# vita-epfl/CrowdNav

Measured on NVIDIA H100. Metric: env-steps/sec at 5 humans × batched envs; 500-case success/collision parity, higher is better.
Workload: dtype f64 state + f32 ORCA solver

## Files before the change

crowdnav_b200/csrc/orca_spec.cuh:

```cuda
#pragma once
#include "orca_device.cuh"

namespace orca {

template <int M> struct RegLines { V2 p[M], d[M]; };

template <int M>
ORCA_HD __forceinline__ int neighbour_order(const float (&dsq)[M], const bool (&inr)[M], const int (&id)[M], int (&src)[M])
{
    static_assert(M <= 10, "3 bits per position in a 32-bit word");
    int rank[M];
    #pragma unroll
    for (int c = 0; c < M; ++c) rank[c] = 0;
    #pragma unroll
    for (int c = 1; c < M; ++c) {
        #pragma unroll
        for (int cc = 0; cc < c; ++cc) {
            const bool le = dsq[cc] <= dsq[c];
            rank[c] += (inr[cc] && le) ? 1 : 0;
            rank[cc] += (inr[c] && !le) ? 1 : 0;
        }
    }
    int nl = 0; unsigned packed = 0u;
    #pragma unroll
    for (int c = 0; c < M; ++c) if (inr[c]) { packed |= (unsigned)id[c] << (3 * rank[c]); ++nl; }
    #pragma unroll
    for (int kk = 0; kk < M; ++kk) src[kk] = (int)((packed >> (3 * kk)) & 7u);
    return nl;
}

ORCA_HD __forceinline__ void make_line_sel(V2 p, V2 v, float r, V2 po, V2 vo, float ro, float inv_th, float inv_dt,
                                              V2 &point, V2 &dir)
{
    const V2 rel_pos = po - p;
    const V2 rel_vel = v - vo;
    const float dist_sq = abssq(rel_pos);
    const float comb_r = r + ro;
    const float comb_r_sq = sqr(comb_r);
    V2 u;
    if (dist_sq > comb_r_sq) {
        const V2 w = rel_vel - inv_th * rel_pos;
        const float w_len_sq = abssq(w);
        const float dot1 = dot(w, rel_pos);
        const float w_len = sqrtf(w_len_sq);
        const V2 unit_w = vdiv(w, w_len);
        const V2 dir_c = mk(unit_w.y, -unit_w.x);
        const V2 u_c = (comb_r * inv_th - w_len) * unit_w;
        const float leg = sqrtf(dist_sq - comb_r_sq);
        const bool left = det(rel_pos, w) > 0.0f;
        const V2 num_l = mk(rel_pos.x * leg - rel_pos.y * comb_r, rel_pos.x * comb_r + rel_pos.y * leg);
        const V2 num_r = mk(rel_pos.x * leg + rel_pos.y * comb_r, -rel_pos.x * comb_r + rel_pos.y * leg);
        const V2 q = vdiv(left ? num_l : num_r, dist_sq);
        const V2 dir_l = left ? q : -q;
        const float dot2 = dot(rel_vel, dir_l);
        const V2 u_l = dot2 * dir_l - rel_vel;
        const bool cutoff = dot1 < 0.0f && sqr(dot1) > comb_r_sq * w_len_sq;
        dir = cutoff ? dir_c : dir_l;
        u = cutoff ? u_c : u_l;
    } else {
        const V2 w = rel_vel - inv_dt * rel_pos;
        const float w_len = sqrtf(abssq(w));
        const V2 unit_w = vdiv(w, w_len);
        dir = mk(unit_w.y, -unit_w.x);
        u = (comb_r * inv_dt - w_len) * unit_w;
    }
    point = v + 0.5f * u;
}

template <int M, int CNT>
ORCA_HD __forceinline__ void lp1_all(const RegLines<M> &R, const bool (&valid)[M], float radius, V2 opt, bool dir_opt,
                                        V2 (&cand)[M], bool (&feas)[M])
{
    #pragma unroll
    for (int i = 0; i < CNT; ++i) {
        const V2 lp = R.p[i], ld = R.d[i];
        const float dp = dot(lp, ld);
        const float disc = sqr(dp) + sqr(radius) - abssq(lp);
        const float sq = sqrtf(disc);
        float t_left = -dp - sq, t_right = -dp + sq;
        bool bad = disc < 0.0f;
        #pragma unroll
        for (int j = 0; j < i; ++j) {
            const float den = det(ld, R.d[j]);
            const float num = det(R.d[j], lp - R.p[j]);
            const bool use = valid[j];
            const bool par = fabsf(den) <= kEps;
            const bool live_pair = use && !par;
            const float t = (live_pair ? num : 1.0f) / (live_pair ? den : 1.0f);
            bad = bad || (use && par && num < 0.0f);
            const bool right = use && !par && den >= 0.0f, leftb = use && !par && den < 0.0f;
            t_right = (right && t < t_right) ? t : t_right;
            t_left = (leftb && t_left < t) ? t : t_left;
        }
        feas[i] = !bad && !(t_left > t_right);
        if (dir_opt) {
            cand[i] = (dot(opt, ld) > 0.0f) ? (lp + t_right * ld) : (lp + t_left * ld);
        } else {
            const float t = dot(ld, opt - lp);
            const float tc = (t < t_left) ? t_left : ((t > t_right) ? t_right : t);
            cand[i] = lp + tc * ld;
        }
    }
}

template <int M, int CNT>
ORCA_HD __forceinline__ int lp2_scan(const RegLines<M> &R, const bool (&valid)[M], int count, const V2 (&cand)[M], const bool (&feas)[M],
                                        V2 init, V2 &result)
{
    result = init;
    int fail = count;
    #pragma unroll
    for (int i = 0; i < CNT; ++i) {
        const bool viol = (i < count) && (fail == count) && valid[i] && det(R.d[i], R.p[i] - result) > 0.0f;
        if (viol) { if (!feas[i]) fail = i; else result = cand[i]; }
    }
    return fail;
}

ORCA_HD __forceinline__ V2 lp2_init(V2 opt, float radius)
{
    if (abssq(opt) > sqr(radius)) { const V2 nv = normalize(opt); return mk(nv.x * radius, nv.y * radius); }
    return opt;
}

ORCA_HD __forceinline__ float int_bits(int i) { float f; __builtin_memcpy(&f, &i, sizeof f); return f; }
ORCA_HD __forceinline__ int bits_int(float f) { int i; __builtin_memcpy(&i, &f, sizeof i); return i; }

template <int M>
struct Lp3Queue {
    static constexpr int kLines = M, kRows = 4 * M + 3;
    float *base;
    int stride;
    ORCA_HD __forceinline__ Lines lines(int col) const { return { base + col, stride }; }
    ORCA_HD __forceinline__ int n(int col) const { return bits_int(base[(4 * M + 0) * stride + col]); }
    ORCA_HD __forceinline__ int fail(int col) const { return bits_int(base[(4 * M + 1) * stride + col]); }
    ORCA_HD __forceinline__ float radius(int col) const { return base[(4 * M + 2) * stride + col]; }
    ORCA_HD __forceinline__ void put(int col, const RegLines<M> &R, int nl, int fail, float radius) const
    {
        #pragma unroll
        for (int kk = 0; kk < M; ++kk) lines(col).set(kk, R.p[kk], R.d[kk]);
        base[(4 * M + 0) * stride + col] = int_bits(nl); base[(4 * M + 1) * stride + col] = int_bits(fail);
        base[(4 * M + 2) * stride + col] = radius;
    }
};

#define ORCA_LP3_SUBPROBLEM_LANE(Q, COL, I, P, R2, RS, C) do {                                                         \
        const orca::Lines lq_ = (Q).lines(COL);                                                                          \
        const int qn_ = (Q).n(COL);                                                                                      \
        bool ok_ = false; orca::V2 r_ = orca::mk(0.f, 0.f);                                                             \
        if ((Q).kLines > 1 && (I) < qn_) ok_ = orca::lp3_subproblem(lq_, (I), (Q).radius(COL), (P), r_);                \
        (R2)[C] = r_.x; (R2)[(RS) + (C)] = r_.y; (R2)[2 * (RS) + (C)] = ok_ ? 1.0f : 0.0f;                             \
    } while (0)
#define ORCA_LP3_SCAN_LANE(Q, COL, RES, R2, RS, C) do {                                                                \
        const int qn_ = (Q).n(COL), qf_ = (Q).fail(COL);                                                                 \
        const float qr_ = (Q).radius(COL);                                                                               \
        orca::lp3_outer_scan((Q).lines(COL), qn_, qf_, qr_, (RES), [&](int ii_, orca::V2 &r_) {                         \
            const int src_ = (C) + (ii_ - 1);                                                                            \
            r_ = orca::mk((R2)[src_], (R2)[(RS) + src_]);                                                                \
            return (R2)[2 * (RS) + src_] != 0.0f;                                                                        \
        });                                                                                                              \
    } while (0)

template <int M>
ORCA_HD __forceinline__ void insert_sorted(float dd, int j, float (&td)[M], int (&tj)[M])
{
    #pragma unroll
    for (int kk = M - 1; kk >= 0; --kk) {
        const int km = kk > 0 ? kk - 1 : 0;
        const bool lt = dd < td[kk];
        const bool ltp = (kk > 0) && (dd < td[km]);
        td[kk] = ltp ? td[km] : (lt ? dd : td[kk]);
        tj[kk] = ltp ? tj[km] : (lt ? j : tj[kk]);
    }
}

}
```

crowdnav_b200/csrc/step_multi.cuh:

```cuda
#pragma once
#include "step_flat.cuh"
#include "rotate.cuh"

namespace cs {

#ifndef CS_MULTI_WARPS
#define CS_MULTI_WARPS 30
#endif

#define CS_PHASES 8
#ifdef CS_PHASE_PROBE
static __device__ unsigned long long g_phase[2][CS_PHASES + 1];
#define CS_PROBE_INIT unsigned ph_acc[CS_PHASES] = {}; long long ph_t = clock64();
#define CS_PROBE(i) do { const long long t_ = clock64(); ph_acc[i] += (unsigned)(t_ - ph_t); ph_t = t_; } while (0)
#define CS_PROBE_FLUSH(robot, steps) do { if ((threadIdx.x & 31) == 0) {                                                    \
        for (int i_ = 0; i_ < CS_PHASES; ++i_) atomicAdd(&g_phase[(robot) ? 1 : 0][i_], (unsigned long long)ph_acc[i_]);    \
        atomicAdd(&g_phase[(robot) ? 1 : 0][CS_PHASES], (unsigned long long)(steps)); } } while (0)
#else
#define CS_PROBE_INIT
#define CS_PROBE(i) do { } while (0)
#define CS_PROBE_FLUSH(robot, steps) do { } while (0)
#endif

template <int N, int M, bool ROBOT>
__device__ __forceinline__ orca::V2 multi_solve(const KParams &k, const float4 *s_view, const float *s_rview, int ebase, int a,
                                                bool solves, double2 pos, double2 goal, double v_pref, orca::V2 p, orca::V2 v,
                                                float r, const float *s_rl, orca::RegLines<N> &Rq, int &nl_out, int &fail_out,
                                                float &max_speed_out)
{
    using namespace orca;
    const V2 pref = pref_velocity(pos, goal);
    const float max_speed = (float)v_pref;

    float dsq[M]; bool inr[M]; int jj[M], src[M];
    #pragma unroll
    for (int c = 0; c < M; ++c) {
        const int j = ROBOT ? c : ((c < N - 1) ? ((c < a) ? c : c + 1) : N);
        jj[c] = j;
        const float4 q = s_view[ebase + j];
        dsq[c] = abssq(p - mk(q.x, q.y));
        inr[c] = solves && (k.max_neighbors > 0) && dsq[c] < sqr(k.neighbor_dist);
    }
    int nl = neighbour_order<M>(dsq, inr, jj, src);
    nl = nl < k.max_neighbors ? nl : k.max_neighbors;

    constexpr int T = 32 * (N + 1);
    if (ROBOT) asm volatile("barrier.sync 1, %0;" :: "r"(T) : "memory");
    RegLines<M> R; bool valid[M];
    #pragma unroll
    for (int kk = 0; kk < M; ++kk) {
        valid[kk] = kk < nl;
        R.p[kk] = mk(0.f, 0.f); R.d[kk] = mk(0.f, 0.f);
        if (valid[kk]) {
            if (ROBOT) {
                const int c = (ebase / (N + 1)) * N + src[kk];
                R.p[kk] = mk(s_rl[0 * T + c], s_rl[1 * T + c]); R.d[kk] = mk(s_rl[2 * T + c], s_rl[3 * T + c]);
            } else {
                const int sl = ebase + src[kk];
                const float4 q = s_view[sl];
                make_line_sel(p, v, r, mk(q.x, q.y), mk(q.z, q.w), s_rview[sl], k.inv_time_horizon, k.inv_time_step, R.p[kk], R.d[kk]);
            }
        }
    }

    V2 cand[M]; bool feas[M];
    lp1_all<M, M>(R, valid, max_speed, pref, false, cand, feas);
    V2 nv = mk(0.f, 0.f);
    fail_out = lp2_scan<M, M>(R, valid, nl, cand, feas, lp2_init(pref, max_speed), nv);
    #pragma unroll
    for (int kk = 0; kk < N; ++kk) { Rq.p[kk] = (kk < M) ? R.p[kk] : mk(0.f, 0.f); Rq.d[kk] = (kk < M) ? R.d[kk] : mk(0.f, 0.f); }
    nl_out = nl; max_speed_out = max_speed;
    return nv;
}

template <int E>
__device__ __forceinline__ float *rec_vpref_smem()
{
    __shared__ float s_vp[E];
    return s_vp;
}

template <int E>
__device__ __forceinline__ float *rec_theta_smem()
{
    __shared__ float s_th[E];
    return s_th;
}

template <bool ROT = false>
__device__ __forceinline__ void rec_row(const crowdsim_record &rec, int B, int N, int s, int e, int a, double2 hp, double2 hv,
                                        double hr, double2 rp, double2 rv, double2 rg, double rr, float rvp, float rth = 0.f)
{
    float c, sn, rot, dg, rvx, rvy;
    rotate_self((float)rp.x, (float)rp.y, (float)rv.x, (float)rv.y, (float)rg.x, (float)rg.y, c, sn, rot, dg, rvx, rvy);
    float row[13];
    rotate_row(row, (float)rp.x, (float)rp.y, (float)rr, rvp, ROT ? (rth - rot) : 0.f, dg, rvx, rvy, c, sn, (float)hp.x,
               (float)hp.y, (float)hv.x, (float)hv.y, (float)hr);
    float *o = rec.rows + (((size_t)s * B + e) * N + a) * 13;
    #pragma unroll
    for (int i = 0; i < 13; ++i) o[i] = row[i];
}

__device__ __forceinline__ void rec_map_state(const crowdsim_record_maps &m, int B, int N, int s, int e, int a, double2 hp, double2 hv)
{
    const size_t i = ((size_t)s * B + e) * N + a;
    st2(m.h_pos, i, hp); st2(m.h_vel, i, hv);
}

template <int N, bool VIS, bool REC, bool ROT = false, bool ARR = false, bool MET = false>
__global__ void __launch_bounds__(32 * (N + 1), CS_MULTI_WARPS / (N + 1))
step_multi_kernel(const __grid_constant__ StepArgs A)
{
    static_assert(REC || !ROT, "unicycle rows are a recording variant");
    static_assert(!(REC && ARR), "arrivals are stamped by the rollout kernels only");
    static_assert(!(REC && MET), "metrics are measured by the rollout kernels only");
    static_assert(N >= 2 && N <= 5, "small crowds with at least two humans (N = 1 runs n single-step launches)");
    using namespace orca;
    CS_RES_BEGIN
    constexpr int E = 32, L = N + 1, T = 32 * L;
    constexpr int MH = VIS ? N : N - 1;
    constexpr int SUB = N - 1;
    constexpr int IPW = 32 / SUB;
    constexpr int QC = IPW * L;
    constexpr int QF = Lp3Queue<N>::kRows + 1;
    constexpr int PV = (4 * SUB > 10) ? 4 * SUB : 10;
    __shared__ float s_q[QF][QC];
    __shared__ __align__(16) float s_pv[PV][T];
    __shared__ __align__(16) float s_r2[3][T];
    __shared__ double2 s_pos[T], s_vel[T];
    __shared__ double2 s_goal[T];
    __shared__ double s_rad[T];
    __shared__ float2 s_nv[T];
    __shared__ RobotRec s_rr[E];
    __shared__ uint8_t s_pre[E];
    __shared__ int s_qcount;
    constexpr unsigned PRE_TIMEOUT = 1, PRE_GOAL = 2, PRE_READY = 4, PRE_WANT = 8;
    float4 *const s_view = reinterpret_cast<float4 *>(&s_pv[0][0]);
    float *const s_radh = s_pv[4], *const s_radr = s_pv[5];
    const Lp3Queue<N> Q = { &s_q[0][0], QC };

    const KParams &k = A.k;
    const int tid = threadIdx.x;
    const bool is_robot = tid >= 32 * N;
    const int le = is_robot ? tid - 32 * N : tid / N;
    const int a = is_robot ? N : tid - le * N;
    const int slot_me = le * L + a;
    const int e = blockIdx.x * E + le;
    const bool env_ok = e < A.B;
    const size_t hi = (size_t)e * N + a;
    if (tid == 0) s_qcount = 0;

    double2 pos = make_double2(0, 0), vel = pos, goal = make_double2(3, 4), attr = make_double2(0.3, 1.0);
    uint8_t act_flag = 1;
    if (env_ok) {
        if (A.st.active) act_flag = A.st.active[e];
        if (!is_robot) {
            pos = ld2(A.st.h_pos, hi); vel = ld2(A.st.h_vel, hi); goal = ld2(A.st.h_goal, hi); attr = ld2(A.st.h_attr, hi);
        } else {
            pos = ld2(A.st.r_pos, e); vel = ld2(A.st.r_vel, e); goal = ld2(A.st.r_goal, e); attr = ld2(A.st.r_attr, e);
            RobotRec r0 = {}; r0.ep_c = -1;
            r0.gtime = A.st.g_time[e];
            if (A.has_ep) { r0.ep_t = A.ep.ep_steps[e]; r0.ep_ret = A.ep.ep_return[e]; r0.ep_tc = A.ep.ep_too_close[e]; r0.ep_mds = A.ep.ep_min_dist_sum[e]; r0.ep_c = A.ep.ep_case[e]; }
            if (A.has_ar) r0.want = A.ar.want[e];
            s_rr[le] = r0;
            if constexpr (ROT) rec_theta_smem<E>()[le] = (float)A.st.r_theta[e];
            if constexpr (MET) met_acc_smem<E>()[le] = met_load(A.met, e);
        }
    }
    if constexpr (MET) { if (is_robot) met_hh_smem<E>()[le] = 0; }
    s_goal[tid] = goal;
    RobotRec &rr = s_rr[le];
    bool arrived = false;
    if constexpr (ARR) { if (env_ok && !is_robot) arrived = A.arr.h_arrival[hi] != 0.0; }

    bool dirty_kin = false, dirty_scene = false;
    bool release = false;
    const double dt = k.time_step;
    CS_PROBE_INIT

    #pragma unroll 1
    for (int s = 0; ; ++s) {
    const bool live = env_ok && (act_flag != 0);
    const float fpx = (float)pos.x, fpy = (float)pos.y, fvx = (float)vel.x, fvy = (float)vel.y;
    const float frh = orca_radius(attr.x, k.human_safety_space);
    const float frr = orca_radius(attr.x, k.robot_safety_space);
    s_view[slot_me] = make_float4(fpx, fpy, fvx, fvy); s_radh[slot_me] = frh; s_radr[slot_me] = frr;
    s_pos[tid] = pos; s_vel[tid] = vel; s_rad[tid] = attr.x;
    if constexpr (REC) { if (is_robot) rec_vpref_smem<E>()[le] = (float)attr.y; }
    const bool work = live || (is_robot && env_ok && A.has_ar && rr.want != 0);
    const int go = __syncthreads_or(s < A.n_steps && work);
    if (release) { st_release_u8(A.ar.n_state + e, CROWDSIM_SLOT_EMPTY); release = false; }
    if (!go) {
        if constexpr (REC) { if (is_robot && env_ok) for (int s2 = s; s2 < A.n_steps; ++s2) A.rec.code[(size_t)s2 * A.B + e] = CROWDSIM_REC_NONE; }
        CS_PROBE_FLUSH(is_robot, s);
        break;
    }
    CS_PROBE(0);
    if constexpr (REC) {
        if (!is_robot && live) {
            const int rt = 32 * N + le;
            if constexpr (ROT)
                rec_row<true>(A.rec, A.B, N, s, e, a, pos, vel, attr.x, s_pos[rt], s_vel[rt], s_goal[rt], s_rad[rt],
                              rec_vpref_smem<E>()[le], rec_theta_smem<E>()[le]);
            else
                rec_row(A.rec, A.B, N, s, e, a, pos, vel, attr.x, s_pos[rt], s_vel[rt], s_goal[rt], s_rad[rt], rec_vpref_smem<E>()[le]);
            if (A.recm.h_pos) rec_map_state(A.recm, A.B, N, s, e, a, pos, vel);
        }
    }

    const V2 p = mk(fpx, fpy), v = mk(fvx, fvy);
    if (!is_robot) {
        const int rs = le * L + N;
        const float4 q = s_view[rs];
        V2 lp, ld;
        make_line_sel(mk(q.x, q.y), mk(q.z, q.w), s_radr[rs], p, v, frr, k.inv_time_horizon, k.inv_time_step, lp, ld);
        s_pv[6][tid] = lp.x; s_pv[7][tid] = lp.y; s_pv[8][tid] = ld.x; s_pv[9][tid] = ld.y;
        asm volatile("barrier.arrive 1, %0;" :: "r"(T) : "memory");
    }
    RegLines<N> R; int nl, fail; float max_speed;
    V2 nv = is_robot ? multi_solve<N, N, true>(k, s_view, s_radr, le * L, N, live, pos, s_goal[tid], attr.y, p, v, frr, s_pv[6], R, nl, fail, max_speed)
                     : multi_solve<N, MH, false>(k, s_view, s_radh, le * L, a, live, pos, s_goal[tid], attr.y, p, v, frh, s_pv[6], R, nl, fail, max_speed);

    const bool pending = live && fail < nl;
    int slot = pending ? atomicAdd(&s_qcount, 1) : -1;
    if (slot >= QC) {
        float lq[4 * N], lp[4 * SUB];
        #pragma unroll
        for (int kk = 0; kk < N; ++kk) { lq[4 * kk + 0] = R.p[kk].x; lq[4 * kk + 1] = R.p[kk].y; lq[4 * kk + 2] = R.d[kk].x; lq[4 * kk + 3] = R.d[kk].y; }
        const Lines Lq = { lq, 1 }, Pq = { lp, 1 };
        lp3(Lq, nl, fail, max_speed, Pq, nv);
        slot = -1;
    } else if (slot >= 0) {
        Q.put(slot, R, nl, fail, max_speed); s_q[QF - 1][slot] = __int_as_float(tid);
    }
    s_nv[tid] = make_float2(nv.x, nv.y);
    uint8_t sst = CROWDSIM_SLOT_EMPTY;
    double disc = 0.0;
    if (is_robot && env_ok) {
        if (A.has_ar) sst = ld_relaxed_u8(A.ar.n_state + e);
        if (A.has_ep && live) { const int t = rr.ep_t; disc = (t < A.ep.discount_len) ? A.ep.discount[t] : 0.0; }
    }
    CS_PROBE(1);
    const int cnt = __syncthreads_count(slot >= 0);
    CS_PROBE(2);
    if (cnt > 0) {
        if (tid == 0) s_qcount = 0;
        const int lane = tid & 31, item = (tid >> 5) * IPW + lane / SUB, i = lane % SUB + 1;
        const bool mine = lane < IPW * SUB && item < cnt;
        if (mine) { const Lines Pq = { &s_pv[0][tid], T }; ORCA_LP3_SUBPROBLEM_LANE(Q, item, i, Pq, &s_r2[0][0], T, tid); }
        __syncwarp();
        if (mine && i == 1) {
            const int owner = __float_as_int(s_q[QF - 1][item]);
            const float2 r0 = s_nv[owner];
            V2 res = mk(r0.x, r0.y);
            ORCA_LP3_SCAN_LANE(Q, item, res, &s_r2[0][0], T, tid);
            s_nv[owner] = make_float2(res.x, res.y);
        }
        __syncthreads();
        if (slot >= 0) { const float2 q = s_nv[tid]; nv = mk(q.x, q.y); }
    }
    pos = s_pos[tid]; vel = s_vel[tid];
    CS_PROBE(3);

    double *const s_cl = reinterpret_cast<double *>(&s_r2[0][0]);
    bool timeout = false, reaching_goal = false;
    int arr_c = -1;
    if (!is_robot) {
        if (live) {
            const int rt = 32 * N + le;
            const float2 rv = s_nv[rt];
            s_cl[tid] = swept_clearance(pos, vel, s_pos[rt], make_double2((double)rv.x, (double)rv.y), attr.x, s_rad[rt], dt);
            if constexpr (MET) {
                int c = 0;
                #pragma unroll
                for (int j = 1; j < N; ++j) if (j > a) c += hh_overlap(pos, attr.x, s_pos[le * N + j], s_rad[le * N + j]) ? 1 : 0;
                if (c) atomicAdd(&met_hh_smem<E>()[le], c);
            }
            const double hx = (double)nv.x, hy = (double)nv.y;
            pos = make_double2(pos.x + hx * dt, pos.y + hy * dt); vel = make_double2(hx, hy);
            dirty_kin = true;
            if constexpr (ARR) {
                arr_c = rr.ep_c;
                const double2 g = s_goal[tid];
                if (!arrived && norm2(pos.x - g.x, pos.y - g.y) < attr.x) { A.arr.h_arrival[hi] = rr.gtime + dt; arrived = true; }
            }
        }
    } else if (env_ok) {
        if (live) {
            const double npx = pos.x + (double)nv.x * dt, npy = pos.y + (double)nv.y * dt;
            const double2 goal = s_goal[tid];
            reaching_goal = norm2(npx - goal.x, npy - goal.y) < attr.x;
            timeout = rr.gtime >= k.time_limit - 1;
        }
        s_pre[le] = (uint8_t)((timeout ? PRE_TIMEOUT : 0u) | (reaching_goal ? PRE_GOAL : 0u) |
                              (sst == CROWDSIM_SLOT_READY ? PRE_READY : 0u) | (rr.want != 0 ? PRE_WANT : 0u));
    }
    CS_PROBE(4);
    __syncthreads();
    CS_PROBE(5);
    if (!is_robot) {
        if (env_ok) {
            const unsigned pf = s_pre[le];
            bool done = false;
            if (live) {
                bool collision = false;
                #pragma unroll
                for (int i = 0; i < N; ++i) collision |= s_cl[le * N + i] < 0;
                done = (pf & PRE_TIMEOUT) || collision || (pf & PRE_GOAL);
                if (done && A.has_ep && A.st.active && !A.has_ar) act_flag = 0;
                if constexpr (ARR) {
                    if (done && arr_c >= 0) arr_snap_human(A, arr_c, N, a, pos, vel, s_goal[tid], attr, arrived ? A.arr.h_arrival[hi] : 0.0);
                }
            }
            if (A.has_ar && ((live && done) || (!live && (pf & PRE_WANT)))) {
                act_flag = (pf & PRE_READY) ? 1 : 0;
                if (act_flag) {
                    (void)ld_acquire_u8(A.ar.n_state + e);
                    pos = ld2_cg(A.ar.n_h_pos, hi); vel = make_double2(0, 0); s_goal[tid] = ld2_cg(A.ar.n_h_goal, hi); attr = ld2_cg(A.ar.n_h_attr, hi);
                    dirty_kin = true; dirty_scene = true;
                    if constexpr (ARR) { A.arr.h_arrival[hi] = 0.0; arrived = false; }
                }
            }
        }
        CS_PROBE(6);
    } else {
        if (env_ok) {
            bool done = false;
            if (live) {
                const double ax = (double)nv.x, ay = (double)nv.y;
                double dmin = __longlong_as_double(0x7ff0000000000000LL); bool collision = false;
                #pragma unroll
                for (int i = 0; i < N; ++i) {
                    const double ci = s_cl[le * N + i];
                    if (!collision) { if (ci < 0) collision = true; else if (ci < dmin) dmin = ci; }
                }
                const double npx = pos.x + ax * dt, npy = pos.y + ay * dt;
                if constexpr (MET) {
                    int &hh = met_hh_smem<E>()[le];
                    met_add(met_acc_smem<E>()[le], pos, make_double2(npx, npy), dmin, hh);
                    hh = 0;
                }
                const double gtime = rr.gtime;
                const int t_rec = rr.ep_t;
                double reward;
                const int info = reward_ladder(timeout, collision, reaching_goal, dmin, k, dt, reward);
                done = ends_episode(info);
                pos = make_double2(npx, npy); vel = make_double2(ax, ay);
                const double ntime = gtime + dt;
                rr.gtime = ntime;
                rr.o_act = vel; rr.o_reward = reward; rr.o_dmin = dmin; rr.o_done = done ? 1 : 0; rr.o_info = info; rr.any_live = 1;
                dirty_kin = true;
                if (A.has_ep) {
                    const crowdsim_episodes &ep = A.ep;
                    int ep_t = rr.ep_t, ep_tc = rr.ep_tc; double ep_ret = rr.ep_ret, ep_mds = rr.ep_mds;
                    ep_ret = ep_ret + disc * reward; ep_t += 1;
                    if (info == CROWDSIM_INFO_DANGER) { ep_tc += 1; ep_mds += dmin; }
                    rr.ep_t = ep_t; rr.ep_tc = ep_tc; rr.ep_ret = ep_ret; rr.ep_mds = ep_mds;
                    rr.dirty_ep = 1;
                    if (done) {
                        const int ep_c = rr.ep_c;
                        if (ep_c >= 0) {
                            ep.res_info[ep_c] = (uint8_t)info; ep.res_steps[ep_c] = ep_t;
                            ep.res_time[ep_c] = (info == CROWDSIM_INFO_TIMEOUT) ? k.time_limit : ntime;
                            ep.res_return[ep_c] = ep_ret; ep.res_too_close[ep_c] = ep_tc; ep.res_min_dist_sum[ep_c] = ep_mds;
                            if (ep.res_final_rpos) st2(ep.res_final_rpos, ep_c, pos);
                            if constexpr (ARR) { if (A.arr.snap_r_vel) st2(A.arr.snap_r_vel, ep_c, vel); }
                            if constexpr (MET) met_result(A.met, ep_c, met_acc_smem<E>()[le]);
                        }
                        if (A.st.active && !A.has_ar) { A.st.active[e] = 0; act_flag = 0; }
                    }
                }
                if constexpr (REC) {
                    const size_t ri = (size_t)s * A.B + e;
                    A.rec.reward[ri] = reward; A.rec.t[ri] = t_rec;
                    A.rec.code[ri] = !done ? CROWDSIM_REC_LIVE : (info == CROWDSIM_INFO_TIMEOUT) ? CROWDSIM_REC_DROPPED : CROWDSIM_REC_STORED;
                }
            } else if constexpr (REC) {
                A.rec.code[(size_t)s * A.B + e] = CROWDSIM_REC_NONE;
            }
            if (A.has_ar) {
                const bool finished = live && done, parked = !live && rr.want != 0;
                if (finished || parked) {
                    if (sst == CROWDSIM_SLOT_READY) {
                        (void)ld_acquire_u8(A.ar.n_state + e);
                        pos = make_double2(0.0, -A.ar.circle_radius); s_goal[tid] = make_double2(0.0, A.ar.circle_radius);
                        vel = make_double2(0, 0); attr = make_double2(A.ar.robot_radius, A.ar.robot_v_pref);
                        rr.gtime = 0.0;
                        if (A.st.r_theta) A.st.r_theta[e] = CS_PI / 2;
                        if constexpr (ROT) rec_theta_smem<E>()[le] = (float)A.st.r_theta[e];
                        if (A.has_ep) { rr.ep_t = 0; rr.ep_ret = 0.0; rr.ep_tc = 0; rr.ep_mds = 0.0; rr.ep_c = __ldcg(A.ar.n_case + e); rr.dirty_ep = 1; rr.new_case = 1; }
                        if constexpr (MET) met_acc_smem<E>()[le] = met_fresh();
                        act_flag = 1; A.st.active[e] = 1; rr.want = 0; A.ar.want[e] = 0;
                        dirty_kin = true; dirty_scene = true; release = true;
                    } else {
                        act_flag = 0; A.st.active[e] = 0;
                        const uint8_t want = (sst == CROWDSIM_SLOT_EXHAUSTED) ? 0 : 1;
                        rr.want = want; A.ar.want[e] = want;
                    }
                }
            }
        }
        CS_PROBE(6);
    }
    }

    if (env_ok) {
        if (!is_robot) {
            if (dirty_kin) {
                st2(A.st.h_pos, hi, pos); st2(A.st.h_vel, hi, vel);
                if (A.io.obs32) reinterpret_cast<float4 *>(A.io.obs32)[hi] = make_float4((float)pos.x, (float)pos.y, (float)vel.x, (float)vel.y);
            }
            if (dirty_scene) { st2(A.st.h_goal, hi, s_goal[tid]); st2(A.st.h_attr, hi, attr); }
        } else {
            if (dirty_kin) { st2(A.st.r_pos, e, pos); st2(A.st.r_vel, e, vel); A.st.g_time[e] = rr.gtime; }
            if (dirty_scene) { st2(A.st.r_goal, e, s_goal[tid]); st2(A.st.r_attr, e, attr); }
            if (rr.any_live) {
                if (A.io.action_out) st2(A.io.action_out, e, rr.o_act);
                A.io.reward[e] = rr.o_reward; A.io.dmin[e] = rr.o_dmin; A.io.done[e] = rr.o_done; A.io.info[e] = (uint8_t)rr.o_info;
            }
            if (A.has_ep && rr.dirty_ep) {
                A.ep.ep_steps[e] = rr.ep_t; A.ep.ep_return[e] = rr.ep_ret; A.ep.ep_too_close[e] = rr.ep_tc; A.ep.ep_min_dist_sum[e] = rr.ep_mds;
                if (rr.new_case) A.ep.ep_case[e] = rr.ep_c;
                if constexpr (MET) met_store(A.met, e, met_acc_smem<E>()[le]);
            }
        }
    }
    CS_RES_END(CS_RES_STEP);
}

}
```

Baseline: 1.338 billion.

## Share symmetric pairwise ORCA core terms between human pairs via shared-memory table

Splits ORCA line construction into a symmetric pair core (overlap/cutoff decision, leg length and reciprocal, with flags packed into sign bits) and a per-agent finish. Each human pair's core is now computed once and written to a shared-memory table for both agents, so the sqrt and divide are not repeated per direction. Human neighbour lines are then built from the table. This adds a named barrier across the human threads, extra shared-memory traffic and a dependence on the core being exactly symmetric. It also aliases s_r2 and the table into the s_pv shared-memory allocation to save space.

```diff
diff --git a/crowdnav_b200/csrc/orca_spec.cuh b/crowdnav_b200/csrc/orca_spec.cuh
--- a/crowdnav_b200/csrc/orca_spec.cuh
+++ b/crowdnav_b200/csrc/orca_spec.cuh
@@ -67,6 +67,58 @@
     point = v + 0.5f * u;
 }
 
+ORCA_HD __forceinline__ float int_bits(int i) { float f; __builtin_memcpy(&f, &i, sizeof f); return f; }
+ORCA_HD __forceinline__ int bits_int(float f) { int i; __builtin_memcpy(&i, &f, sizeof i); return i; }
+
+ORCA_HD __forceinline__ V2 pair_core(V2 p, V2 v, float r, V2 po, V2 vo, float ro, float inv_th, float inv_dt)
+{
+    const V2 rel_pos = po - p;
+    const V2 rel_vel = v - vo;
+    const float dist_sq = abssq(rel_pos);
+    const float comb_r = r + ro;
+    const float comb_r_sq = sqr(comb_r);
+    const bool overlap = !(dist_sq > comb_r_sq);
+    const V2 w = rel_vel - (overlap ? inv_dt : inv_th) * rel_pos;
+    const float w_len_sq = abssq(w);
+    const float dot1 = dot(w, rel_pos);
+    const bool circle = overlap || (dot1 < 0.0f && sqr(dot1) > comb_r_sq * w_len_sq);
+    const bool left = det(rel_pos, w) > 0.0f;
+    const float len = sqrtf(circle ? w_len_sq : dist_sq - comb_r_sq);
+    const float inv = 1.0f / (circle ? len : dist_sq);
+    return mk(circle ? -len : len, (circle ? overlap : left) ? -inv : inv);
+}
+
+ORCA_HD __forceinline__ void line_from_core(V2 c, V2 p, V2 v, float r, V2 po, V2 vo, float ro, float inv_th, float inv_dt,
+                                            V2 &point, V2 &dir)
+{
+    const bool circle = bits_int(c.x) < 0, flag = bits_int(c.y) < 0;
+    const float len = fabsf(c.x), inv = fabsf(c.y);
+    const V2 rel_pos = po - p;
+    const V2 rel_vel = v - vo;
+    const float comb_r = r + ro;
+    const float k = (circle && flag) ? inv_dt : inv_th;
+    const V2 w = rel_vel - k * rel_pos;
+    const V2 unit_w = mk(w.x * inv, w.y * inv);
+    const V2 dir_c = mk(unit_w.y, -unit_w.x);
+    const V2 u_c = (comb_r * k - len) * unit_w;
+    const V2 num_l = mk(rel_pos.x * len - rel_pos.y * comb_r, rel_pos.x * comb_r + rel_pos.y * len);
+    const V2 num_r = mk(rel_pos.x * len + rel_pos.y * comb_r, -rel_pos.x * comb_r + rel_pos.y * len);
+    const V2 n = flag ? num_l : num_r;
+    const V2 q = mk(n.x * inv, n.y * inv);
+    const V2 dir_l = flag ? q : -q;
+    const float dot2 = dot(rel_vel, dir_l);
+    const V2 u_l = dot2 * dir_l - rel_vel;
+    dir = circle ? dir_c : dir_l;
+    const V2 u = circle ? u_c : u_l;
+    point = v + 0.5f * u;
+}
+
+ORCA_HD __forceinline__ void make_line_core(V2 p, V2 v, float r, V2 po, V2 vo, float ro, float inv_th, float inv_dt,
+                                            V2 &point, V2 &dir)
+{
+    line_from_core(pair_core(p, v, r, po, vo, ro, inv_th, inv_dt), p, v, r, po, vo, ro, inv_th, inv_dt, point, dir);
+}
+
 template <int M, int CNT>
 ORCA_HD __forceinline__ void lp1_all(const RegLines<M> &R, const bool (&valid)[M], float radius, V2 opt, bool dir_opt,
                                         V2 (&cand)[M], bool (&feas)[M])
@@ -123,9 +175,6 @@
     return opt;
 }
 
-ORCA_HD __forceinline__ float int_bits(int i) { float f; __builtin_memcpy(&f, &i, sizeof f); return f; }
-ORCA_HD __forceinline__ int bits_int(float f) { int i; __builtin_memcpy(&i, &f, sizeof i); return i; }
-
 template <int M>
 struct Lp3Queue {
     static constexpr int kLines = M, kRows = 4 * M + 3;
diff --git a/crowdnav_b200/csrc/step_multi.cuh b/crowdnav_b200/csrc/step_multi.cuh
--- a/crowdnav_b200/csrc/step_multi.cuh
+++ b/crowdnav_b200/csrc/step_multi.cuh
@@ -22,11 +22,18 @@
 #define CS_PROBE_FLUSH(robot, steps) do { } while (0)
 #endif
 
+template <int S>
+__device__ __forceinline__ float2 *pair_table_smem()
+{
+    __shared__ float2 s_pt[S];
+    return s_pt;
+}
+
 template <int N, int M, bool ROBOT>
 __device__ __forceinline__ orca::V2 multi_solve(const KParams &k, const float4 *s_view, const float *s_rview, int ebase, int a,
                                                 bool solves, double2 pos, double2 goal, double v_pref, orca::V2 p, orca::V2 v,
-                                                float r, const float *s_rl, orca::RegLines<N> &Rq, int &nl_out, int &fail_out,
-                                                float &max_speed_out)
+                                                float r, const float *s_rl, const float2 *s_pt, orca::RegLines<N> &Rq,
+                                                int &nl_out, int &fail_out, float &max_speed_out)
 {
     using namespace orca;
     const V2 pref = pref_velocity(pos, goal);
@@ -56,9 +63,15 @@
                 const int c = (ebase / (N + 1)) * N + src[kk];
                 R.p[kk] = mk(s_rl[0 * T + c], s_rl[1 * T + c]); R.d[kk] = mk(s_rl[2 * T + c], s_rl[3 * T + c]);
             } else {
-                const int sl = ebase + src[kk];
+                const int b = src[kk], sl = ebase + b;
                 const float4 q = s_view[sl];
-                make_line_sel(p, v, r, mk(q.x, q.y), mk(q.z, q.w), s_rview[sl], k.inv_time_horizon, k.inv_time_step, R.p[kk], R.d[kk]);
+                if (M == N && b == N) {
+                    make_line_core(p, v, r, mk(q.x, q.y), mk(q.z, q.w), s_rview[sl], k.inv_time_horizon, k.inv_time_step, R.p[kk], R.d[kk]);
+                } else {
+                    const float2 c = s_pt[b];
+                    line_from_core(mk(c.x, c.y), p, v, r, mk(q.x, q.y), mk(q.z, q.w), s_rview[sl], k.inv_time_horizon,
+                                   k.inv_time_step, R.p[kk], R.d[kk]);
+                }
             }
         }
     }
@@ -125,8 +138,8 @@
     constexpr int QF = Lp3Queue<N>::kRows + 1;
     constexpr int PV = (4 * SUB > 10) ? 4 * SUB : 10;
     __shared__ float s_q[QF][QC];
-    __shared__ __align__(16) float s_pv[PV][T];
-    __shared__ __align__(16) float s_r2[3][T];
+    __shared__ __align__(16) float s_pv[PV + 3][T];
+    float (*const s_r2)[T] = s_pv + PV;
     __shared__ double2 s_pos[T], s_vel[T];
     __shared__ double2 s_goal[T];
     __shared__ double s_rad[T];
@@ -137,6 +150,9 @@
     constexpr unsigned PRE_TIMEOUT = 1, PRE_GOAL = 2, PRE_READY = 4, PRE_WANT = 8;
     float4 *const s_view = reinterpret_cast<float4 *>(&s_pv[0][0]);
     float *const s_radh = s_pv[4], *const s_radr = s_pv[5];
+    float2 *s_pt;
+    if constexpr ((PV + 3 - 10) * T >= 2 * E * N * N) s_pt = reinterpret_cast<float2 *>(&s_pv[10][0]);
+    else s_pt = pair_table_smem<E * N * N>();
     const Lp3Queue<N> Q = { &s_q[0][0], QC };
 
     const KParams &k = A.k;
@@ -213,13 +229,25 @@
         const int rs = le * L + N;
         const float4 q = s_view[rs];
         V2 lp, ld;
-        make_line_sel(mk(q.x, q.y), mk(q.z, q.w), s_radr[rs], p, v, frr, k.inv_time_horizon, k.inv_time_step, lp, ld);
+        make_line_core(mk(q.x, q.y), mk(q.z, q.w), s_radr[rs], p, v, frr, k.inv_time_horizon, k.inv_time_step, lp, ld);
         s_pv[6][tid] = lp.x; s_pv[7][tid] = lp.y; s_pv[8][tid] = ld.x; s_pv[9][tid] = ld.y;
         asm volatile("barrier.arrive 1, %0;" :: "r"(T) : "memory");
+        if (live) {
+            #pragma unroll 1
+            for (int d = 1; d <= N / 2; ++d) {
+                if (2 * d < N || a < d) {
+                    const int b = (a + d < N) ? a + d : a + d - N, sl = le * L + b;
+                    const float4 qb = s_view[sl];
+                    const V2 c = pair_core(p, v, frh, mk(qb.x, qb.y), mk(qb.z, qb.w), s_radh[sl], k.inv_time_horizon, k.inv_time_step);
+                    s_pt[tid * N + b] = make_float2(c.x, c.y); s_pt[(le * N + b) * N + a] = make_float2(c.x, c.y);
+                }
+            }
+        }
+        asm volatile("barrier.sync 2, %0;" :: "r"(32 * N) : "memory");
     }
     RegLines<N> R; int nl, fail; float max_speed;
-    V2 nv = is_robot ? multi_solve<N, N, true>(k, s_view, s_radr, le * L, N, live, pos, s_goal[tid], attr.y, p, v, frr, s_pv[6], R, nl, fail, max_speed)
-                     : multi_solve<N, MH, false>(k, s_view, s_radh, le * L, a, live, pos, s_goal[tid], attr.y, p, v, frh, s_pv[6], R, nl, fail, max_speed);
+    V2 nv = is_robot ? multi_solve<N, N, true>(k, s_view, s_radr, le * L, N, live, pos, s_goal[tid], attr.y, p, v, frr, s_pv[6], s_pt, R, nl, fail, max_speed)
+                     : multi_solve<N, MH, false>(k, s_view, s_radh, le * L, a, live, pos, s_goal[tid], attr.y, p, v, frh, s_pv[6], s_pt + tid * N, R, nl, fail, max_speed);
 
     const bool pending = live && fail < nl;
     int slot = pending ? atomicAdd(&s_qcount, 1) : -1;
```

After: 1.397 billion (median of 6 runs). 4.4% higher.
